# mratsim/constantine

Measured on AMD Instinct MI355X. Metric: MSM points/sec, BLS12-381 G1, 2^20 random pairs; pipelined throughput, 2 MSMs in flight, inputs resident in HBM, higher is better.
Workload: dtype u32; 1 GPU; bls12_381_g1 MSM, 2^20 (scalar,point) pairs per GPU, inputs resident in HBM, 2 MSMs in flight (BASELINE.json configs[1]); pairs_per_gpu=1048576, total_pairs=1048576, ranks=1, scalar_bits=255, window_bits=16, windows=16, entries_per_lane=131, seed=1592590338

## Files before the change

constantine_amd/csrc/msm_engine.hip:

```cpp
#include <memory>
#include <mutex>
#include <atomic>
#include <system_error>
#include <thread>
#include <vector>

#if defined(__linux__)
#include <pthread.h>
#include <sched.h>
#endif

#include "hip_backend.h"

using namespace ctt;

#include <stdarg.h>
namespace ctt {
ErrorState& error_state() {
  static thread_local ErrorState st;
  return st;
}
void set_last_error(int code, const char* fmt, ...) {
  ErrorState& st = error_state();
  st.code = code;
  va_list ap;
  va_start(ap, fmt);
  vsnprintf(st.msg, sizeof st.msg, fmt, ap);
  va_end(ap);
}
void hip_failed(const char* expr, const char* what, int is_oom, const char* file, int line) {
  const char* base = strrchr(file, '/');
  set_last_error(is_oom ? ERR_OUT_OF_MEMORY : ERR_HIP_FAILURE, "%s -> %s (%s:%d)", expr, what, base ? base + 1 : file, line);
  (void)hipGetLastError();
  if (error_state().guard > 0) throw HipFailure{error_state().code};
  fprintf(stderr, "[ctt_msm_hip] FATAL %s (no error channel on this path: aborting)\n", error_state().msg);
  abort();
}
DeviceScope::DeviceScope(int device) : dev(device) {
  if (hipGetDevice(&prev) != hipSuccess) {
    (void)hipGetLastError();
    prev = -1;
  }
  if (prev != dev) {
    const hipError_t e = hipSetDevice(dev);
    if (e != hipSuccess) hip_failed("hipSetDevice(context's device)", hipGetErrorString(e), 0, __FILE__, __LINE__);
  }
}
DeviceScope::~DeviceScope() {
  if (prev >= 0 && prev != dev) (void)hipSetDevice(prev);
}
}

extern "C" {
#pragma GCC visibility push(default)
void ctt_hip_msm_ctx_destroy(struct ctt_hip_msm_ctx* ctx);
#pragma GCC visibility pop
const CurveOps* ctt_ops_bls12_381_g1(void);
const CurveOps* ctt_ops_bls12_381_g2(void);
const CurveOps* ctt_ops_bn254_snarks_g1(void);
const CurveOps* ctt_ops_bn254_snarks_g2(void);
const CurveOps* ctt_ops_pallas(void);
const CurveOps* ctt_ops_vesta(void);
const CurveOps* ctt_ops_banderwagon(void);
}

static constexpr uint32_t GS_LDS_WORDS = 39936;
static constexpr uint32_t GS_RPT = 20;
static constexpr uint32_t GS_MAXBG = 1024;
static constexpr uint32_t ENTRY_INVALID = 0xffffffffu;

__device__ __forceinline__ void load_scalar(const uint32_t* __restrict__ scalars, uint32_t j, uint32_t* k) {
  const uint4* p = reinterpret_cast<const uint4*>(scalars + 8ull * j);
  uint4 lo = p[0], hi = p[1];
  k[0] = lo.x; k[1] = lo.y; k[2] = lo.z; k[3] = lo.w;
  k[4] = hi.x; k[5] = hi.y; k[6] = hi.z; k[7] = hi.w;
}

__device__ __forceinline__ uint32_t sort_gshift(const SortArgs& a, uint32_t w) { return a.lay.is_wide(w) ? a.gshift : a.gshift_narrow; }
__device__ __forceinline__ uint32_t sort_group(const SortArgs& a, uint32_t w, uint32_t b) {
  const uint32_t g = b >> sort_gshift(a, w);
  return g < a.NG ? g : a.NG - 1u;
}

static constexpr int PA_NS = 4;
static constexpr int PS_NS = 4;
template <int NS>
__device__ __forceinline__ void load_scalars(const SortArgs& a, uint32_t jb, uint32_t j1, uint32_t (&k)[NS][8]) {
#pragma unroll
  for (int s = 0; s < NS; s++) {
    const uint32_t j = jb + (uint32_t)s * blockDim.x + threadIdx.x;
    if (j < j1) {
      load_scalar(a.scalars, j, k[s]);
    } else {
#pragma unroll
      for (int q = 0; q < 8; q++) k[s][q] = 0u;
    }
  }
}
__device__ __forceinline__ uint32_t part_slice_of_block(const SortArgs& a, uint32_t b, uint32_t nblk) {
  if (!a.xcd_map) return b;
  const uint32_t q = nblk >> 3, r = nblk & 7u, x = b & 7u;
  return x * q + (x < r ? x : r) + (b >> 3);
}
__global__ void __launch_bounds__(512) k_part_count(SortArgs a, uint32_t w0, uint32_t nw) {
  extern __shared__ uint32_t lds[];
  const uint32_t ncnt = a.merged ? a.NG : nw * a.NG;
  const uint32_t wstep = a.merged ? 0u : a.NG;
  for (uint32_t i = threadIdx.x; i < ncnt; i += blockDim.x) lds[i] = 0;
  if (blockIdx.x == 0 && w0 == 0 && threadIdx.x < 4) a.maxcount[threadIdx.x] = 0;
  __syncthreads();
  const uint32_t blk = part_slice_of_block(a, blockIdx.x, gridDim.x);
  const uint32_t j0 = blk * a.slice;
  const uint32_t j1 = (j0 + a.slice < a.n) ? j0 + a.slice : a.n;
  for (uint32_t jb = j0; jb < j1; jb += PA_NS * blockDim.x) {
    uint32_t k[PA_NS][8];
    load_scalars<PA_NS>(a, jb, j1, k);
    for_each_digit<PA_NS>(k, w0, nw, a.lay, [&](uint32_t w, const uint32_t (&d)[PA_NS]) {
#pragma unroll
      for (int s = 0; s < PA_NS; s++)
        if (d[s] != DIGIT_NONE) atomicAdd(&lds[(w - w0) * wstep + sort_group(a, w, d[s] >> 1)], 1u);
    });
  }
  __syncthreads();
  uint32_t* out = a.cntA + (uint64_t)blk * (a.W * a.NG) + (uint64_t)(a.merged ? 0u : w0) * a.NG;
  for (uint32_t i = threadIdx.x; i < ncnt; i += blockDim.x) out[i] = lds[i];
}

static constexpr uint32_t SCAN_CX = 16, SCAN_RG = 64;
__global__ void __launch_bounds__(1024) k_part_scan_blocks(uint32_t* __restrict__ cntA, uint32_t* __restrict__ gtot,
                                                           uint32_t ncol, uint32_t nblk) {
  __shared__ uint32_t part[SCAN_RG][SCAN_CX];
  const uint32_t cx = threadIdx.x % SCAN_CX, rg = threadIdx.x / SCAN_CX;
  const uint32_t col = blockIdx.x * SCAN_CX + cx;
  const uint32_t R = (nblk + SCAN_RG - 1u) / SCAN_RG;
  const uint32_t r0 = rg * R < nblk ? rg * R : nblk, r1 = (r0 + R < nblk) ? r0 + R : nblk;
  uint32_t sum = 0;
  if (col < ncol)
    for (uint32_t r = r0; r < r1; r++) sum += cntA[(uint64_t)r * ncol + col];
  part[rg][cx] = sum;
  __syncthreads();
  uint32_t run = 0, tot = 0;
  for (uint32_t g = 0; g < SCAN_RG; g++) {
    const uint32_t v = part[g][cx];
    if (g < rg) run += v;
    tot += v;
  }
  if (col < ncol) {
    for (uint32_t r = r0; r < r1; r++) {
      uint32_t* p = cntA + (uint64_t)r * ncol + col;
      const uint32_t v = *p;
      *p = run;
      run += v;
    }
    if (rg == 0) gtot[col] = tot;
  }
}

__global__ void __launch_bounds__(1024) k_scan_u32(const uint32_t* __restrict__ in, uint32_t* __restrict__ out, uint32_t len) {
  __shared__ uint32_t wsum[16];
  __shared__ uint32_t carry_s;
  const uint32_t tid = threadIdx.x, lane = tid & 63u, wv = tid >> 6;
  const uint32_t* src = in + (uint64_t)blockIdx.x * len;
  uint32_t* dst = out + (uint64_t)blockIdx.x * (len + 1);
  if (tid == 0) carry_s = 0;
  __syncthreads();
  for (uint32_t b0 = 0; b0 < len; b0 += 1024u) {
    const uint32_t b = b0 + tid;
    const uint32_t v = b < len ? src[b] : 0u;
    uint32_t x = v;
#pragma unroll
    for (uint32_t off = 1; off < 64; off <<= 1) {
      const uint32_t y = __shfl_up(x, off, 64);
      if (lane >= off) x += y;
    }
    if (lane == 63) wsum[wv] = x;
    __syncthreads();
    uint32_t base = carry_s;
    for (uint32_t k = 0; k < wv; k++) base += wsum[k];
    if (b < len) dst[b] = base + x - v;
    __syncthreads();
    if (tid == 1023) carry_s = base + x;
    __syncthreads();
  }
  if (tid == 0) dst[len] = carry_s;
}

template <bool MERGED>
__global__ void __launch_bounds__(1024) k_part_scatter(SortArgs a, uint32_t w0, uint32_t nw) {
  extern __shared__ uint32_t lds[];
  const uint32_t ncnt = MERGED ? a.NG : nw * a.NG;
  const uint32_t wstep = MERGED ? 0u : a.NG;
  uint32_t* cur = lds;
  const uint32_t set0 = MERGED ? 0u : w0;
  const uint32_t blk = part_slice_of_block(a, blockIdx.x, gridDim.x);
  const uint32_t* off = a.cntA + (uint64_t)blk * (a.W * a.NG) + (uint64_t)set0 * a.NG;
  for (uint32_t i = threadIdx.x; i < ncnt; i += blockDim.x) {
    const uint32_t w = i / a.NG, g = i - w * a.NG;
    cur[i] = off[i] + a.gbase[(uint64_t)(set0 + w) * (a.NG + 1) + g];
  }
  __syncthreads();
  const uint32_t j0 = blk * a.slice;
  const uint32_t j1 = (j0 + a.slice < a.n) ? j0 + a.slice : a.n;
  const uint32_t sh = a.jbits + 1u;
  for (uint32_t jb = j0; jb < j1; jb += PS_NS * blockDim.x) {
    uint32_t k[PS_NS][8];
    load_scalars<PS_NS>(a, jb, j1, k);
    for_each_digit<PS_NS>(k, w0, nw, a.lay, [&](uint32_t w, const uint32_t (&d)[PS_NS]) {
      __syncthreads();
      uint32_t* cw = cur + (w - w0) * wstep;
      const uint32_t gmask = (1u << sort_gshift(a, w)) - 1u;
      const uint32_t id0 = jb + threadIdx.x;
      uint32_t pos[PS_NS];
#pragma unroll
      for (int s = 0; s < PS_NS; s++) pos[s] = d[s] != DIGIT_NONE ? atomicAdd(&cw[sort_group(a, w, d[s] >> 1)], 1u) : 0u;
      if constexpr (MERGED) {
        uint64_t* pw = reinterpret_cast<uint64_t*>(a.part);
        const uint32_t row0 = w * a.id_stride + id0;
#pragma unroll
        for (int s = 0; s < PS_NS; s++)
          if (d[s] != DIGIT_NONE)
            pw[pos[s]] = ((uint64_t)((d[s] >> 1) & gmask) << 32) | ((d[s] & 1u) << 31) | (row0 + (uint32_t)s * blockDim.x);
      } else {
        uint32_t* pw = a.part + (uint64_t)w * a.nent;
#pragma unroll
        for (int s = 0; s < PS_NS; s++)
          if (d[s] != DIGIT_NONE)
            pw[pos[s]] = (((d[s] >> 1) & gmask) << sh) | ((d[s] & 1u) << a.jbits) | (id0 + (uint32_t)s * blockDim.x);
      }
    });
  }
}

template <bool MERGED>
__global__ void __launch_bounds__(1024) k_part_scatter_staged(SortArgs a) {
  extern __shared__ uint32_t lds[];
  using R = typename std::conditional<MERGED, uint64_t, uint32_t>::type;
  constexpr uint32_t STEP = PS_NS * 1024u;
  const uint32_t NG = a.NG;
  uint32_t* hist = lds;
  uint32_t* lbase = hist + NG;
  uint32_t* gposd = lbase + NG;
  uint32_t* wsum = gposd + NG;
  uint16_t* stage_g = reinterpret_cast<uint16_t*>(wsum + 16);
  R* stage_rec = reinterpret_cast<R*>(stage_g + STEP);
  const uint32_t tid = threadIdx.x, lane = tid & 63u, wv = tid >> 6;
  const uint32_t blk = part_slice_of_block(a, blockIdx.x, gridDim.x);
  uint32_t* cursor = a.cntA + (uint64_t)blk * (a.W * NG);
  if (tid < NG) {
    for (uint32_t set = 0; set < a.W; set++) cursor[set * NG + tid] += a.gbase[(uint64_t)set * (NG + 1) + tid];
    hist[tid] = 0;
  }
  const uint32_t j0 = blk * a.slice;
  const uint32_t j1 = (j0 + a.slice < a.n) ? j0 + a.slice : a.n;
  const uint32_t sh = a.jbits + 1u;
  for (uint32_t jb = j0; jb < j1; jb += STEP) {
    uint32_t k[PS_NS][8];
    load_scalars<PS_NS>(a, jb, j1, k);
    for_each_digit<PS_NS>(k, 0u, a.Wd, a.lay, [&](uint32_t w, const uint32_t (&d)[PS_NS]) {
      const uint32_t set = MERGED ? 0u : w;
      const uint32_t gmask = (1u << sort_gshift(a, w)) - 1u;
      const uint32_t id0 = jb + tid;
      __syncthreads();
      uint32_t g[PS_NS], rk[PS_NS];
#pragma unroll
      for (int s = 0; s < PS_NS; s++) {
        g[s] = d[s] != DIGIT_NONE ? sort_group(a, w, d[s] >> 1) : 0u;
        rk[s] = d[s] != DIGIT_NONE ? atomicAdd(&hist[g[s]], 1u) : 0u;
      }
      __syncthreads();
      const uint32_t v = tid < NG ? hist[tid] : 0u;
      uint32_t x = v;
#pragma unroll
      for (uint32_t o = 1; o < 64; o <<= 1) {
        const uint32_t y = __shfl_up(x, o, 64);
        if (lane >= o) x += y;
      }
      if (lane == 63) wsum[wv] = x;
      __syncthreads();
      uint32_t base = x - v, total = 0;
#pragma unroll
      for (uint32_t q = 0; q < 16; q++) {
        const uint32_t t = wsum[q];
        if (q < wv) base += t;
        total += t;
      }
      if (tid < NG) {
        lbase[tid] = base;
        uint32_t* cp = cursor + set * NG + tid;
        const uint32_t gp = *cp;
        gposd[tid] = gp - base;
        *cp = gp + v;
        hist[tid] = 0;
      }
      __syncthreads();
#pragma unroll
      for (int s = 0; s < PS_NS; s++)
        if (d[s] != DIGIT_NONE) {
          const uint32_t slot = lbase[g[s]] + rk[s];
          stage_g[slot] = (uint16_t)g[s];
          if constexpr (MERGED) {
            stage_rec[slot] = ((uint64_t)((d[s] >> 1) & gmask) << 32) | ((d[s] & 1u) << 31) | (w * a.id_stride + id0 + (uint32_t)s * 1024u);
          } else {
            stage_rec[slot] = (((d[s] >> 1) & gmask) << sh) | ((d[s] & 1u) << a.jbits) | (id0 + (uint32_t)s * 1024u);
          }
        }
      __syncthreads();
      R* pw = reinterpret_cast<R*>(a.part) + (MERGED ? 0ull : (uint64_t)w * a.nent);
      for (uint32_t i = tid; i < total; i += 1024u) pw[gposd[stage_g[i]] + i] = stage_rec[i];
    });
  }
}

template <bool MERGED>
__global__ void __launch_bounds__(1024) k_group_sort(SortArgs a) {
  extern __shared__ uint32_t lds[];
  __shared__ uint32_t wtot[16];
  __shared__ uint32_t wmax[16];
  __shared__ uint32_t any_big;
  __shared__ uint32_t next_tile;
  const uint32_t w = blockIdx.x / a.NG, g = blockIdx.x - w * a.NG;
  const uint32_t gs = sort_gshift(a, w);
  const uint32_t Bg = 1u << gs;
  uint32_t* off = lds;
  uint32_t* cur = lds + (Bg + 1);
  uint32_t* arr = cur + Bg;
  const uint32_t GS_CAP = a.cap, GS_BIG = a.big;
  const uint32_t* gb = a.gbase + (uint64_t)w * (a.NG + 1);
  const uint32_t beg = gb[g], ng = gb[g + 1] - beg;
  const uint32_t* rec = a.part + (uint64_t)w * a.nent + beg;
  const uint64_t* rec64 = reinterpret_cast<const uint64_t*>(a.part) + beg;
  uint32_t* ent = a.entries + (uint64_t)w * a.nent + beg;
  const uint32_t tid = threadIdx.x, lane = tid & 63u, wv = tid >> 6;
  const uint32_t sh = a.jbits + 1u, jmask = (1u << a.jbits) - 1u;
  using R = typename std::conditional<MERGED, uint64_t, uint32_t>::type;
  auto load = [&](uint32_t i) -> R { if constexpr (MERGED) return rec64[i]; else return rec[i]; };
  auto bucket_of = [&](R r) -> uint32_t { if constexpr (MERGED) return (uint32_t)(r >> 32); else return r >> sh; };
  auto entry_of = [&](R r) -> uint32_t {
    if constexpr (MERGED) return (uint32_t)r; else return (r & jmask) | (((r >> a.jbits) & 1u) << 31);
  };

  if (tid < Bg) cur[tid] = 0;
  if (tid == 0) any_big = 0;
  __syncthreads();
  const bool in_regs = ng <= GS_RPT * 1024u;
  R rr[GS_RPT];
  uint32_t rk[GS_RPT];
  if (in_regs) {
#pragma unroll
    for (uint32_t q = 0; q < GS_RPT; q++) {
      const uint32_t i = q * 1024u + tid;
      if (i < ng) rr[q] = load(i);
    }
#pragma unroll
    for (uint32_t q = 0; q < GS_RPT; q++)
      if (q * 1024u + tid < ng) rk[q] = atomicAdd(&cur[bucket_of(rr[q])], 1u);
  } else {
    for (uint32_t i = tid; i < ng; i += 1024u) atomicAdd(&cur[bucket_of(load(i))], 1u);
  }
  __syncthreads();
  const uint32_t cnt = tid < Bg ? cur[tid] : 0u;
  uint32_t x = cnt, mx = cnt;
#pragma unroll
  for (uint32_t o = 1; o < 64; o <<= 1) {
    const uint32_t y = __shfl_up(x, o, 64);
    if (lane >= o) x += y;
  }
  if (lane == 63) wtot[wv] = x;
#pragma unroll
  for (uint32_t o = 32; o >= 1; o >>= 1) {
    const uint32_t y = __shfl_xor(mx, o, 64);
    mx = y > mx ? y : mx;
  }
  if (lane == 0) wmax[wv] = mx;
  if (lane == 0 && mx > GS_BIG) any_big = 1;
  __syncthreads();
  uint32_t base = x - cnt;
  for (uint32_t k = 0; k < wv; k++) base += wtot[k];
  if (tid == 0) {
    uint32_t m = 0;
    for (uint32_t k = 0; k < 16; k++) m = wmax[k] > m ? wmax[k] : m;
    if (m) atomicMax(a.maxcount, m);
  }
  if (tid < Bg) {
    off[tid] = base;
    cur[tid] = base;
    a.bstart[(uint64_t)w * (a.B + 1) + ((uint64_t)g << gs) + tid] = beg + base;
  }
  if (tid == 0) off[Bg] = ng;
  if (g == a.NG - 1)
    for (uint32_t b = (a.NG << gs) + tid; b <= a.B; b += 1024u) a.bstart[(uint64_t)w * (a.B + 1) + b] = beg + ng;
  __syncthreads();
  if (a.zero_bytes) {
    const uint32_t CH = a.zero_bytes >> 4;
    uint4* zw = reinterpret_cast<uint4*>((char*)a.zero_base + (uint64_t)w * a.B * a.zero_bytes);
    uint4* zg = zw + ((uint64_t)g << gs) * CH;
    const uint4 z4 = make_uint4(0u, 0u, 0u, 0u);
    for (uint32_t i = tid; i < Bg * CH; i += 1024u) {
      const uint32_t b = i / CH;
      if (off[b + 1] == off[b]) zg[i] = z4;
    }
    if (g == a.NG - 1)
      for (uint64_t i = (uint64_t)(a.NG << gs) * CH + tid; i < (uint64_t)a.B * CH; i += 1024u) zw[i] = z4;
  }

  if (in_regs && ng <= GS_CAP && !any_big) {
#pragma unroll
    for (uint32_t q = 0; q < GS_RPT; q++)
      if (q * 1024u + tid < ng) arr[off[bucket_of(rr[q])] + rk[q]] = entry_of(rr[q]);
    __syncthreads();
    for (uint32_t p = tid; p < ng; p += 1024u) ent[p] = arr[p];
    return;
  }

  if (any_big) {
    for (uint32_t i = tid; i < ng; i += 1024u) {
      const R r = load(i);
      const uint32_t b = bucket_of(r);
      if (off[b + 1] - off[b] > GS_BIG) ent[atomicAdd(&cur[b], 1u)] = entry_of(r);
    }
  }
  const uint32_t my_cnt = tid < Bg ? off[tid + 1] - off[tid] : 0u;
  const uint32_t my_tile = (my_cnt > 0 && my_cnt <= GS_BIG) ? off[tid] / GS_CAP : 0xffffffffu;
  uint32_t t_prev = 0xffffffffu;
  for (;;) {
    __syncthreads();
    if (tid == 0) next_tile = 0xffffffffu;
    __syncthreads();
    if (my_tile != 0xffffffffu && (t_prev == 0xffffffffu || my_tile > t_prev)) atomicMin(&next_tile, my_tile);
    __syncthreads();
    const uint32_t t = next_tile;
    if (t == 0xffffffffu) break;
    t_prev = t;
    const uint32_t tbase = t * GS_CAP;
    const uint32_t lim = (ng - tbase < GS_CAP + GS_BIG) ? ng - tbase : GS_CAP + GS_BIG;
    for (uint32_t p = tid; p < lim; p += 1024u) arr[p] = ENTRY_INVALID;
    __syncthreads();
    for (uint32_t i = tid; i < ng; i += 1024u) {
      const R r = load(i);
      const uint32_t b = bucket_of(r);
      const uint32_t o = off[b];
      if (off[b + 1] - o <= GS_BIG && o >= tbase && o - tbase < GS_CAP) arr[atomicAdd(&cur[b], 1u) - tbase] = entry_of(r);
    }
    __syncthreads();
    for (uint32_t p = tid; p < lim; p += 1024u) {
      const uint32_t v = arr[p];
      if (v != ENTRY_INVALID) ent[tbase + p] = v;
    }
  }
}

static void pin_thread_to_device_node(int device);

void HipBackend::init(int dev) {
  device = dev;
  HIP_CHECK(hipSetDevice(dev));
  hipDeviceProp_t prop;
  HIP_CHECK(hipGetDeviceProperties(&prop, dev));
  num_cu = prop.multiProcessorCount;
  {
    const char* e;
    if ((e = getenv("CTT_HIP_MSM_QUAD"))) quad_adds = (uint32_t)atoi(e);
    if ((e = getenv("CTT_HIP_MSM_TAIL"))) tail_adds = (uint32_t)atoi(e);
    cu_tail = (e = getenv("CTT_HIP_CU_TAIL")) ? atoi(e) : 0;
    if (cu_tail < 0 || XCDS * cu_tail >= num_cu || num_cu % XCDS != 0) cu_tail = 0;
    cu_main = cu_tail > 0 && !((e = getenv("CTT_HIP_CU_MAIN")) && atoi(e) == 0);
  }
  if (cu_tail > 0) {
    const uint32_t words = ((uint32_t)num_cu + 31u) / 32u;
    std::vector<uint32_t> tail_mask(words, 0u), main_mask(words, 0u);
    for (int b = 0; b < num_cu; b++) (b < XCDS * cu_tail ? tail_mask : main_mask)[b / 32] |= 1u << (b % 32);
    HIP_CHECK(hipExtStreamCreateWithCUMask(&aux, words, tail_mask.data()));
    if (cu_main) HIP_CHECK(hipExtStreamCreateWithCUMask(&stream, words, main_mask.data()));
    else HIP_CHECK(hipStreamCreateWithFlags(&stream, hipStreamNonBlocking));
    own_stream = true;
  } else {
    HIP_CHECK(hipStreamCreateWithFlags(&stream, hipStreamNonBlocking));
    own_stream = true;
    int lo = 0, hi = 0;
    HIP_CHECK(hipDeviceGetStreamPriorityRange(&lo, &hi));
    HIP_CHECK(hipStreamCreateWithPriority(&aux, hipStreamNonBlocking, hi));
  }
  HIP_CHECK(hipStreamCreateWithFlags(&cpy, hipStreamNonBlocking));
  srt = cpy;
  HIP_CHECK(hipEventCreateWithFlags(&ev_accum_done, hipEventDisableTiming));
  HIP_CHECK(hipEventCreateWithFlags(&ev_front_done, hipEventDisableTiming));
  HIP_CHECK(hipEventCreateWithFlags(&ev_copy, hipEventDisableTiming));
  for (int i = 0; i < MAX_CHUNKS; i++) HIP_CHECK(hipEventCreateWithFlags(&ev_slice[i], hipEventDisableTiming));
  for (int i = 0; i < MAX_CHUNKS; i++) HIP_CHECK(hipEventCreateWithFlags(&ev_coefs[i], hipEventDisableTiming));
  HIP_CHECK(hipEventCreateWithFlags(&ev_tail_fork, hipEventDisableTiming));
  HIP_CHECK(hipEventCreateWithFlags(&ev_tail_done, hipEventDisableTiming));
  HIP_CHECK(hipEventCreateWithFlags(&ev_wide_done, hipEventDisableTiming));
  for (int s = 0; s < NSLOT; s++) {
    for (int i = 0; i < ST_COUNT; i++) {
      for (int ch = 0; ch < MAX_CHUNKS; ch++) {
        HIP_CHECK(hipEventCreate(&ev_begin[s][i][ch]));
        HIP_CHECK(hipEventCreate(&ev_end[s][i][ch]));
      }
      ev_used[s][i] = 0;
    }
    HIP_CHECK(hipEventCreateWithFlags(&ev_done[s], hipEventDisableTiming));
  }
  for (int i = 0; i < ST_COUNT; i++) stage_ms[i] = 0.f;
  no_tail = getenv("CTT_HIP_MSM_NO_TAIL") && atoi(getenv("CTT_HIP_MSM_NO_TAIL")) != 0;
  HIP_CHECK(hipFuncSetAttribute((const void*)k_group_sort<false>, hipFuncAttributeMaxDynamicSharedMemorySize,
                                (int)(GS_LDS_WORDS * 4)));
  HIP_CHECK(hipFuncSetAttribute((const void*)k_group_sort<true>, hipFuncAttributeMaxDynamicSharedMemorySize,
                                (int)(GS_LDS_WORDS * 4)));
}

void HipBackend::shutdown() noexcept {
  auto ev = [](hipEvent_t& e) {
    if (e && hipEventDestroy(e) != hipSuccess) (void)hipGetLastError();
    e = nullptr;
  };
  auto st = [](hipStream_t& s) {
    if (s && hipStreamDestroy(s) != hipSuccess) (void)hipGetLastError();
    s = nullptr;
  };
  if (!own_stream) return;
  ev(ev_accum_done); ev(ev_front_done); ev(ev_copy); ev(ev_tail_fork); ev(ev_tail_done); ev(ev_wide_done);
  for (int i = 0; i < MAX_CHUNKS; i++) { ev(ev_slice[i]); ev(ev_coefs[i]); }
  for (int s = 0; s < NSLOT; s++) {
    for (int i = 0; i < ST_COUNT; i++)
      for (int ch = 0; ch < MAX_CHUNKS; ch++) { ev(ev_begin[s][i][ch]); ev(ev_end[s][i][ch]); }
    ev(ev_done[s]);
  }
  srt = nullptr;
  st(cpy); st(aux); st(stream);
  own_stream = false;
}

void HipBackend::launch_digits_sort(const SortArgs& a) {
  const uint32_t ncol = a.W * a.NG;
  if (a.NG > 16384u || a.B / a.NG > GS_MAXBG || 2u * (a.B / a.NG) + 1u + a.cap + a.big > GS_LDS_WORDS ||
      (!a.merged && a.jbits + 1u + a.gshift > 32u) || (a.merged && (a.W != 1 || a.gshift_narrow != a.gshift))) {
    fprintf(stderr, "[ctt_msm_hip] FATAL: sort plan out of range (n = %u, c = %d, groups = %u)\n", a.n, a.c, a.NG);
    abort();
  }
  uint32_t wb = a.merged ? a.Wd : 16384u / a.NG;
  if (wb < 1) wb = 1;
  if (wb > a.Wd) wb = a.Wd;
  for (uint32_t w0 = 0; w0 < a.Wd; w0 += wb) {
    const uint32_t nw = (w0 + wb <= a.Wd) ? wb : a.Wd - w0;
    hipLaunchKernelGGL(k_part_count, dim3(a.nblk), dim3(512), (a.merged ? a.NG : (size_t)nw * a.NG) * 4, front(), a, w0, nw);
    HIP_CHECK(hipGetLastError());
  }
  hipLaunchKernelGGL(k_part_scan_blocks, dim3((ncol + SCAN_CX - 1) / SCAN_CX), dim3(1024), 0, front(), a.cntA, a.gtot, ncol, a.nblk);
  HIP_CHECK(hipGetLastError());
  hipLaunchKernelGGL(k_scan_u32, dim3(a.W), dim3(1024), 0, front(), (const uint32_t*)a.gtot, a.gbase, a.NG);
  HIP_CHECK(hipGetLastError());
  if (a.staged && a.NG <= 1024u && (a.NG & (a.NG - 1u)) == 0u) {
    const size_t rec = a.merged ? 8 : 4;
    const size_t lds_bytes = ((size_t)3 * a.NG + 16) * 4 + (size_t)PS_NS * 1024 * (2 + rec);
    if (a.merged) hipLaunchKernelGGL(k_part_scatter_staged<true>, dim3(a.nblk), dim3(1024), lds_bytes, front(), a);
    else hipLaunchKernelGGL(k_part_scatter_staged<false>, dim3(a.nblk), dim3(1024), lds_bytes, front(), a);
    HIP_CHECK(hipGetLastError());
  } else {
    for (uint32_t w0 = 0; w0 < a.Wd; w0 += wb) {
      const uint32_t nw = (w0 + wb <= a.Wd) ? wb : a.Wd - w0;
      if (a.merged) hipLaunchKernelGGL(k_part_scatter<true>, dim3(a.nblk), dim3(1024), (size_t)a.NG * 4, front(), a, w0, nw);
      else hipLaunchKernelGGL(k_part_scatter<false>, dim3(a.nblk), dim3(1024), (size_t)nw * a.NG * 4, front(), a, w0, nw);
      HIP_CHECK(hipGetLastError());
    }
  }
  const uint32_t Bg = a.B / a.NG;
  const size_t lds = ((size_t)2 * Bg + 1 + a.cap + a.big) * 4;
  if (a.merged) hipLaunchKernelGGL(k_group_sort<true>, dim3(a.W * a.NG), dim3(1024), lds, front(), a);
  else hipLaunchKernelGGL(k_group_sort<false>, dim3(a.W * a.NG), dim3(1024), lds, front(), a);
  HIP_CHECK(hipGetLastError());
}

static constexpr int NUM_CURVES = 7;

static const CurveOps* curve_ops(int id) {
  switch (id) {
    case 0: return ctt_ops_bls12_381_g1();
    case 1: return ctt_ops_bls12_381_g2();
    case 2: return ctt_ops_bn254_snarks_g1();
    case 3: return ctt_ops_bn254_snarks_g2();
    case 4: return ctt_ops_pallas();
    case 5: return ctt_ops_vesta();
    case 6: return ctt_ops_banderwagon();
  }
  return nullptr;
}

static bool out_kind_ok(int curve, int out_kind) {
  return out_kind == OUT_AFF || out_kind == OUT_PRJ || (out_kind == OUT_JAC && curve != Banderwagon::ID);
}
static bool is_weierstrass(int curve) { return curve != Banderwagon::ID; }

struct ctt_hip_msm_ctx {
  HipBackend bk;
  std::mutex mu;
  void* engines[NUM_CURVES] = {nullptr};
  void* in_coefs = nullptr;
  size_t in_coefs_cap = 0;
  void* in_points = nullptr;
  size_t in_points_cap = 0;
  MsmOptions opt;
  int last_plan[8] = {0};
  int last_slot = 0;
  hipEvent_t ev_order = nullptr;
  uint64_t pool_gen = 0;
  int host_chunks = 0;
  bool lost = false;
};

static ctt_hip_msm_ctx* make_ctx(int device) {
  int ndev = 0;
  hipError_t e = hipGetDeviceCount(&ndev);
  if (e != hipSuccess || ndev == 0) {
    (void)hipGetLastError();
    set_last_error(ERR_NO_DEVICE, "no HIP device available (%s); this library has no CPU fallback", hipGetErrorString(e));
    return nullptr;
  }
  if (device < 0 || device >= ndev) {
    set_last_error(ERR_NO_DEVICE, "device %d out of range (%d devices)", device, ndev);
    return nullptr;
  }
  ErrorGuard guard;
  ctt_hip_msm_ctx* c = nullptr;
  try {
    DeviceScope device_scope(device);
    c = new ctt_hip_msm_ctx();
    c->bk.init(device);
  } catch (const HipFailure&) {
    delete c;
    return nullptr;
  }
  c->bk.uploader_hook = pin_thread_to_device_node;
  const char* s;
  if ((s = getenv("CTT_HIP_MSM_C"))) c->opt.c = atoi(s);
  if ((s = getenv("CTT_HIP_MSM_K"))) c->opt.K = atoi(s);
  if ((s = getenv("CTT_HIP_MSM_S"))) c->opt.S = atoi(s);
  if ((s = getenv("CTT_HIP_MSM_CHUNKS"))) c->host_chunks = atoi(s);
  if ((s = getenv("CTT_HIP_MSM_HOST_WINDOW_SUMS"))) c->opt.host_window_sums = atoi(s);
  if ((s = getenv("CTT_HIP_MSM_HORNER_BITS"))) c->opt.horner_bits = atoi(s);
  if ((s = getenv("CTT_SORT_XCD"))) c->opt.sort_xcd = atoi(s);
  if ((s = getenv("CTT_SORT_STAGED"))) c->opt.sort_staged = atoi(s);
  if ((s = getenv("CTT_HIP_MSM_MERGE_CHAIN"))) c->opt.merge_chain = atoi(s);
  if ((s = getenv("CTT_HIP_MSM_MERGE_LMAX"))) c->opt.merge_lmax = atoi(s);
  if ((s = getenv("CTT_HIP_MSM_TIMINGS"))) c->bk.timing = atoi(s);
  return c;
}

static ctt_hip_msm_ctx* default_ctx() {
  static std::mutex mu;
  static ctt_hip_msm_ctx* ctx = nullptr;
  std::lock_guard<std::mutex> lock(mu);
  if (!ctx) {
    const char* s = getenv("CTT_HIP_DEVICE");
    ctx = make_ctx(s ? atoi(s) : 0);
  }
  return ctx;
}
static ctt_hip_msm_ctx* usable(ctt_hip_msm_ctx* ctx) {
  if (!ctx) ctx = default_ctx();
  if (!ctx) return nullptr;
  if (ctx->lost) {
    set_last_error(ERR_HIP_FAILURE, "this context was lost to an earlier HIP failure (device %d); destroy it and create a new one", ctx->bk.device);
    return nullptr;
  }
  return ctx;
}

static constexpr int TICKET_SLOTS = 4;
static int slot_refused(int slot) {
  if (slot == -2) set_last_error(ERR_OUT_OF_MEMORY, "out of device memory while the MSM's workspace was allocated");
  else set_last_error(ERR_BUSY, "three tickets are outstanding on this curve of the context: finish one first");
  return -1;
}
static int msm_device_locked(ctt_hip_msm_ctx* ctx, int curve, void* r_host, int out_kind, const void* d_coefs,
                             bool coef_is_fr, const void* d_points, size_t len) {
  if (len > 0x7fffffffull || !out_kind_ok(curve, out_kind)) return -1;
  const CurveOps* ops = curve_ops(curve);
  DeviceScope device_scope(ctx->bk.device);
  if (!ctx->engines[curve]) ctx->engines[curve] = ops->engine_create(&ctx->bk);
  const int slot = ops->submit(ctx->engines[curve], &ctx->opt, d_coefs, coef_is_fr ? 1 : 0, d_points, (uint32_t)len,
                               ctx->last_plan);
  if (slot < 0) return slot_refused(slot);
  ops->finish(ctx->engines[curve], slot, r_host, out_kind);
  ctx->last_slot = slot;
  return 0;
}

template <class Fn>
static int guarded(Fn&& fn, ctt_hip_msm_ctx** lost_ctx = nullptr) {
  ErrorGuard guard;
  ErrorState& es = error_state();
  es.code = ERR_NONE;
  es.msg[0] = 0;
  try {
    const int rc = fn();
    if (rc < 0 && es.code == ERR_NONE) set_last_error(ERR_REFUSED, "bad arguments (curve id, kind, length, ticket, option key or owner)");
    return rc;
  } catch (const OutOfDeviceMemory& e) {
    set_last_error(ERR_OUT_OF_MEMORY, "out of device memory (%zu bytes requested)", e.bytes);
    return -1;
  } catch (const HipFailure&) {
    if (lost_ctx && *lost_ctx) (*lost_ctx)->lost = true;
    return -1;
  }
}
static void* device_alloc(size_t bytes) {
  void* p = nullptr;
  const hipError_t e = hipMalloc(&p, bytes);
  if (e == hipErrorOutOfMemory) {
    (void)hipGetLastError();
    fprintf(stderr, "[ctt_msm_hip] out of device memory: hipMalloc of %zu bytes failed\n", bytes);
    throw OutOfDeviceMemory{bytes};
  }
  HIP_CHECK(e);
  return p;
}
static void ensure_staging(void*& p, size_t& cap, size_t bytes) {
  if (bytes <= cap) return;
  if (p) HIP_CHECK(hipFree(p));
  p = nullptr;
  cap = 0;
  p = device_alloc(bytes + bytes / 8);
  cap = bytes + bytes / 8;
}

static int msm_host_on_ctx(ctt_hip_msm_ctx* ctx, int curve, void* r, int out_kind, const void* coefs, bool coef_is_fr,
                           const void* points, size_t len) {
  ctx = usable(ctx);
  if (!ctx) return -1;
  if (len > 0x7fffffffull) {
    set_last_error(ERR_REFUSED, "length %zu above 2^31 - 1", len);
    return -1;
  }
  ErrorGuard guard;
  try {
    std::lock_guard<std::mutex> lock(ctx->mu);
    DeviceScope device_scope(ctx->bk.device);
    const CurveOps* ops = curve_ops(curve);
    const size_t cb = len * 32, pb = len * ops->aff_bytes;
    if (len) {
      ensure_staging(ctx->in_coefs, ctx->in_coefs_cap, cb);
      ensure_staging(ctx->in_points, ctx->in_points_cap, pb);
    }
    if (!ctx->engines[curve]) ctx->engines[curve] = ops->engine_create(&ctx->bk);
    const int slot = ops->submit_host(ctx->engines[curve], &ctx->opt, coefs, coef_is_fr ? 1 : 0, points, (uint32_t)len, ctx->in_coefs,
                                      ctx->in_points, ctx->host_chunks, ctx->last_plan);
    if (slot == -2) {
      set_last_error(ERR_OUT_OF_MEMORY, "out of device memory in a host-pointer MSM of %zu pairs", len);
      return -2;
    }
    if (slot < 0) {
      set_last_error(ERR_BUSY, "all in-flight slots of the context are held by tickets of ctt_hip_msm_device_submit");
      return -1;
    }
    ops->finish(ctx->engines[curve], slot, r, out_kind);
    ctx->last_slot = slot;
    return 0;
  } catch (const OutOfDeviceMemory& e) {
    set_last_error(ERR_OUT_OF_MEMORY, "out of device memory (%zu bytes requested)", e.bytes);
    return -2;
  } catch (const HipFailure&) {
    ctx->lost = true;
    return -1;
  }
}

struct ShardSet {
  std::mutex mu;
  int active = 0;
  std::vector<ctt_hip_msm_ctx*> ctxs;
  size_t shard_min = 1u << 15;
  bool env_read = false;
};
static ShardSet& shard_set() {
  static ShardSet s;
  return s;
}

static void shard_set_assign(const int* devices, int n) {
  ShardSet& s = shard_set();
  for (ctt_hip_msm_ctx* c : s.ctxs) ctt_hip_msm_ctx_destroy(c);
  s.ctxs.clear();
  for (int i = 0; i < n; i++) {
    ctt_hip_msm_ctx* c = make_ctx(devices[i]);
    if (c) s.ctxs.push_back(c);
  }
}

static std::vector<ctt_hip_msm_ctx*> shard_contexts(size_t len) {
  ShardSet& s = shard_set();
  std::lock_guard<std::mutex> lock(s.mu);
  if (!s.env_read) {
    s.env_read = true;
    const char* m = getenv("CTT_HIP_SHARD_MIN");
    if (m) s.shard_min = (size_t)strtoull(m, nullptr, 10);
    const char* e = getenv("CTT_HIP_DEVICES");
    if (e && *e && s.ctxs.empty()) {
      std::vector<int> devs;
      if (!strcmp(e, "all")) {
        int nd = 0;
        if (hipGetDeviceCount(&nd) != hipSuccess) { (void)hipGetLastError(); nd = 0; }
        for (int i = 0; i < nd; i++) devs.push_back(i);
      } else {
        for (const char* q = e; *q;) {
          char* end = nullptr;
          long v = strtol(q, &end, 10);
          if (end == q) break;
          devs.push_back((int)v);
          q = (*end == ',') ? end + 1 : end;
        }
      }
      if (devs.size() >= 2) shard_set_assign(devs.data(), (int)devs.size());
    }
  }
  if (s.ctxs.size() < 2 || len < 2 * (s.shard_min ? s.shard_min : 1)) return {};
  size_t g = len / (s.shard_min ? s.shard_min : 1);
  if (g > s.ctxs.size()) g = s.ctxs.size();
  s.active++;
  return std::vector<ctt_hip_msm_ctx*>(s.ctxs.begin(), s.ctxs.begin() + g);
}
static void shard_release() {
  ShardSet& s = shard_set();
  std::lock_guard<std::mutex> lock(s.mu);
  s.active--;
}

static void pin_thread_to_device_node(int device) {
#if defined(__linux__)
  static const bool on = !(getenv("CTT_HIP_NUMA_PIN") && atoi(getenv("CTT_HIP_NUMA_PIN")) == 0);
  if (!on) return;
  char bus[64] = {0};
  if (hipDeviceGetPCIBusId(bus, (int)sizeof(bus) - 1, device) != hipSuccess) { (void)hipGetLastError(); return; }
  for (char* p = bus; *p; p++) if (*p >= 'A' && *p <= 'F') *p = (char)(*p - 'A' + 'a');
  char path[256];
  snprintf(path, sizeof path, "/sys/bus/pci/devices/%s/numa_node", bus);
  FILE* f = fopen(path, "r");
  if (!f) return;
  int node = -1;
  const int got = fscanf(f, "%d", &node);
  fclose(f);
  if (got != 1 || node < 0) return;
  snprintf(path, sizeof path, "/sys/devices/system/node/node%d/cpulist", node);
  f = fopen(path, "r");
  if (!f) return;
  char list[4096] = {0};
  const size_t nr = fread(list, 1, sizeof(list) - 1, f);
  fclose(f);
  if (nr == 0) return;
  cpu_set_t set;
  CPU_ZERO(&set);
  int any = 0;
  for (char* p = list; *p;) {
    char* end = nullptr;
// ... 714 lines not shown
```

Before: 373.5 million points/s.

## Shrink sort scan kernels, batch row loads, and raise wave priority under overlap

The block-offset scan now uses 256-thread blocks over 4 columns, with a column-block swizzle and 8-row batched loads so reads can be in flight together. The per-window group scan becomes a single 64-lane wavefront that holds 3 elements per lane, prefetches the next chunk, and needs no LDS or barriers. Both kernels raise wave priority with s_setprio when tail or wide work is pending on another stream. The aim is to shorten these small serial kernels on the critical path of the pipelined MSM. The cost is less parallelism per scan block, and the priority boost can slow the concurrent kernels.

```diff
diff --git a/constantine_amd/csrc/msm_engine.hip b/constantine_amd/csrc/msm_engine.hip
--- a/constantine_amd/csrc/msm_engine.hip
+++ b/constantine_amd/csrc/msm_engine.hip
@@ -126,63 +126,83 @@
   for (uint32_t i = threadIdx.x; i < ncnt; i += blockDim.x) out[i] = lds[i];
 }
 
-static constexpr uint32_t SCAN_CX = 16, SCAN_RG = 64;
-__global__ void __launch_bounds__(1024) k_part_scan_blocks(uint32_t* __restrict__ cntA, uint32_t* __restrict__ gtot,
-                                                           uint32_t ncol, uint32_t nblk) {
+static constexpr uint32_t SCAN_CX = 4, SCAN_RG = 64, SCAN_ROWS = 8;
+__global__ void __launch_bounds__(SCAN_CX * SCAN_RG) k_part_scan_blocks(uint32_t* __restrict__ cntA, uint32_t* __restrict__ gtot,
+                                                                        uint32_t ncol, uint32_t nblk, uint32_t prio) {
+  if (prio) __builtin_amdgcn_s_setprio(3);
   __shared__ uint32_t part[SCAN_RG][SCAN_CX];
   const uint32_t cx = threadIdx.x % SCAN_CX, rg = threadIdx.x / SCAN_CX;
-  const uint32_t col = blockIdx.x * SCAN_CX + cx;
+  const uint32_t q = gridDim.x >> 3, rem = gridDim.x & 7u, x = blockIdx.x & 7u;
+  const uint32_t col = (x * q + (x < rem ? x : rem) + (blockIdx.x >> 3)) * SCAN_CX + cx;
   const uint32_t R = (nblk + SCAN_RG - 1u) / SCAN_RG;
   const uint32_t r0 = rg * R < nblk ? rg * R : nblk, r1 = (r0 + R < nblk) ? r0 + R : nblk;
   uint32_t sum = 0;
-  if (col < ncol)
-    for (uint32_t r = r0; r < r1; r++) sum += cntA[(uint64_t)r * ncol + col];
+  if (col < ncol) {
+    for (uint32_t r = r0; r < r1; r += SCAN_ROWS) {
+      uint32_t v[SCAN_ROWS];
+#pragma unroll
+      for (uint32_t k = 0; k < SCAN_ROWS; k++) v[k] = r + k < r1 ? cntA[(uint64_t)(r + k) * ncol + col] : 0u;
+#pragma unroll
+      for (uint32_t k = 0; k < SCAN_ROWS; k++) sum += v[k];
+    }
+  }
   part[rg][cx] = sum;
   __syncthreads();
   uint32_t run = 0, tot = 0;
+#pragma unroll 8
   for (uint32_t g = 0; g < SCAN_RG; g++) {
     const uint32_t v = part[g][cx];
     if (g < rg) run += v;
     tot += v;
   }
   if (col < ncol) {
-    for (uint32_t r = r0; r < r1; r++) {
-      uint32_t* p = cntA + (uint64_t)r * ncol + col;
-      const uint32_t v = *p;
-      *p = run;
-      run += v;
+    for (uint32_t r = r0; r < r1; r += SCAN_ROWS) {
+      uint32_t v[SCAN_ROWS];
+#pragma unroll
+      for (uint32_t k = 0; k < SCAN_ROWS; k++) v[k] = r + k < r1 ? cntA[(uint64_t)(r + k) * ncol + col] : 0u;
+#pragma unroll
+      for (uint32_t k = 0; k < SCAN_ROWS; k++) {
+        if (r + k < r1) cntA[(uint64_t)(r + k) * ncol + col] = run;
+        run += v[k];
+      }
     }
     if (rg == 0) gtot[col] = tot;
   }
 }
 
-__global__ void __launch_bounds__(1024) k_scan_u32(const uint32_t* __restrict__ in, uint32_t* __restrict__ out, uint32_t len) {
-  __shared__ uint32_t wsum[16];
-  __shared__ uint32_t carry_s;
-  const uint32_t tid = threadIdx.x, lane = tid & 63u, wv = tid >> 6;
+static constexpr uint32_t SCAN_EPL = 3;
+__global__ void __launch_bounds__(64) k_scan_u32(const uint32_t* __restrict__ in, uint32_t* __restrict__ out, uint32_t len, uint32_t prio) {
+  if (prio) __builtin_amdgcn_s_setprio(3);
+  const uint32_t lane = threadIdx.x;
   const uint32_t* src = in + (uint64_t)blockIdx.x * len;
   uint32_t* dst = out + (uint64_t)blockIdx.x * (len + 1);
-  if (tid == 0) carry_s = 0;
-  __syncthreads();
-  for (uint32_t b0 = 0; b0 < len; b0 += 1024u) {
-    const uint32_t b = b0 + tid;
-    const uint32_t v = b < len ? src[b] : 0u;
-    uint32_t x = v;
+  uint32_t carry = 0, v[SCAN_EPL], nv[SCAN_EPL];
+#pragma unroll
+  for (uint32_t k = 0; k < SCAN_EPL; k++) nv[k] = lane * SCAN_EPL + k < len ? src[lane * SCAN_EPL + k] : 0u;
+  for (uint32_t b0 = 0; b0 < len; b0 += 64u * SCAN_EPL) {
+    const uint32_t b = b0 + lane * SCAN_EPL, bn = b + 64u * SCAN_EPL;
+    uint32_t x = 0;
+#pragma unroll
+    for (uint32_t k = 0; k < SCAN_EPL; k++) {
+      v[k] = nv[k];
+      x += v[k];
+      nv[k] = bn + k < len ? src[bn + k] : 0u;
+    }
+    const uint32_t mine = x;
 #pragma unroll
     for (uint32_t off = 1; off < 64; off <<= 1) {
       const uint32_t y = __shfl_up(x, off, 64);
       if (lane >= off) x += y;
     }
-    if (lane == 63) wsum[wv] = x;
-    __syncthreads();
-    uint32_t base = carry_s;
-    for (uint32_t k = 0; k < wv; k++) base += wsum[k];
-    if (b < len) dst[b] = base + x - v;
-    __syncthreads();
-    if (tid == 1023) carry_s = base + x;
-    __syncthreads();
-  }
-  if (tid == 0) dst[len] = carry_s;
+    uint32_t base = carry + x - mine;
+#pragma unroll
+    for (uint32_t k = 0; k < SCAN_EPL; k++) {
+      if (b + k < len) dst[b + k] = base;
+      base += v[k];
+    }
+    carry += __shfl(x, 63, 64);
+  }
+  if (lane == 0) dst[len] = carry;
 }
 
 template <bool MERGED>
@@ -545,9 +565,11 @@
     hipLaunchKernelGGL(k_part_count, dim3(a.nblk), dim3(512), (a.merged ? a.NG : (size_t)nw * a.NG) * 4, front(), a, w0, nw);
     HIP_CHECK(hipGetLastError());
   }
-  hipLaunchKernelGGL(k_part_scan_blocks, dim3((ncol + SCAN_CX - 1) / SCAN_CX), dim3(1024), 0, front(), a.cntA, a.gtot, ncol, a.nblk);
+  const uint32_t scan_prio = (tail_pending || wide_pending) ? 1u : 0u;
+  hipLaunchKernelGGL(k_part_scan_blocks, dim3((ncol + SCAN_CX - 1) / SCAN_CX), dim3(SCAN_CX * SCAN_RG), 0, front(), a.cntA, a.gtot, ncol,
+                     a.nblk, scan_prio);
   HIP_CHECK(hipGetLastError());
-  hipLaunchKernelGGL(k_scan_u32, dim3(a.W), dim3(1024), 0, front(), (const uint32_t*)a.gtot, a.gbase, a.NG);
+  hipLaunchKernelGGL(k_scan_u32, dim3(a.W), dim3(64), 0, front(), (const uint32_t*)a.gtot, a.gbase, a.NG, scan_prio);
   HIP_CHECK(hipGetLastError());
   if (a.staged && a.NG <= 1024u && (a.NG & (a.NG - 1u)) == 0u) {
     const size_t rec = a.merged ? 8 : 4;
```

Result: no change. 376.8 million points/s, median of 6 (+0.9%).
